# biotite-dev/springcraft

Hardware: AMD Instinct MI355X
Metric: ANM modes/sec (Hessian build + full eigensolve), N=2000 C-alpha (higher is better)
Workload: dtype f64; 1 GPU; C3: N=2000 C-alpha ANM, HinsenForceField (no cutoff), full 6000x6000 eigensolve, all modes + vectors; parallelism=independent structures sharded over GPUs, no data-path collective

## Files before the change

### springcraft_amd/csrc/host_logic.h

```cpp
#pragma once
#include <cmath>
#include <cstdarg>
#include <cstdint>
#include <cstdio>
#include <map>
#include <string>
#include <utility>
#include <vector>

#include "scratch_arena.h"
#include "springcraft_hip.h"

namespace sc_host {

static inline int fail(std::string& err, int code, const char* fmt, ...) {
  char buf[512];
  va_list ap;
  va_start(ap, fmt);
  vsnprintf(buf, sizeof(buf), fmt, ap);
  va_end(ap);
  err = buf;
  return code;
}

static inline int check_ff(const sc_ff_desc* ff, std::string& err) {
  if (!ff) return fail(err, SC_ERR_INVALID_ARG, "force-field descriptor is NULL");
  if (ff->kind < SC_FF_INVARIANT || ff->kind > SC_FF_TABULATED)
    return fail(err, SC_ERR_INVALID_ARG, "unknown force-field kind %d", ff->kind);
  if (ff->kind == SC_FF_TABULATED) {
    const sc_tab_desc* t = ff->tab;
    if (!t || t->n_bins < 1 || !t->bonded || !t->intra_chain || !t->inter_chain || !t->atom_type || !t->chain ||
        !t->bonded_next || (t->n_bins > 1 && !t->edges_sq))
      return fail(err, SC_ERR_INVALID_ARG, "incomplete tabulated force-field descriptor");
  }
  if (ff->kind == SC_FF_INVARIANT && !ff->has_cutoff)
    return fail(err, SC_ERR_INVALID_ARG, "Cutoff distance must be a float");
  return SC_OK;
}

struct HostPatch {
  bool any = false;
  std::vector<uint8_t> shut;
  std::vector<int32_t> row_ptr, col;
  std::vector<int8_t> flag;
  std::vector<double> gam;
  int mask_gamma = 0;
  struct Bufs { uint8_t* shut; int32_t* rp; int32_t* col; int8_t* flag; double* gam; };
  Bufs layout(Arena& a) const {
    return Bufs{a.take<uint8_t>(shut.size()), a.take<int32_t>(row_ptr.size()), a.take<int32_t>(col.size() + 1),
                a.take<int8_t>(flag.size() + 1), a.take<double>(gam.size() + 1)};
  }
  size_t device_bytes() const {
    Arena a;
    layout(a);
    return a.bytes();
  }
};

static inline int build_patch(const sc_patch_desc* pd, int64_t n, HostPatch& hp, std::string& err) {
  hp.any = false;
  if (!pd || (pd->n_shutdown == 0 && pd->n_pair_off == 0 && pd->n_pair_on == 0)) return SC_OK;
  if (pd->n_shutdown < 0 || pd->n_pair_off < 0 || pd->n_pair_on < 0 ||
      (pd->n_shutdown && !pd->shutdown) || (pd->n_pair_off && !pd->pair_off) ||
      (pd->n_pair_on && !pd->pair_on))
    return fail(err, SC_ERR_INVALID_ARG, "inconsistent patch descriptor");
  hp.any = true;
  hp.mask_gamma = pd->base_cutoff_masks_gamma;
  hp.shut.assign((size_t)n, 0);
  auto in_range = [&](int64_t v) { return v >= 0 && v < n; };
  for (int64_t s = 0; s < pd->n_shutdown; ++s) {
    if (!in_range(pd->shutdown[s]))
      return fail(err, SC_ERR_INDEX, "Index %lld is out of bounds for a structure of length %lld",
                          (long long)pd->shutdown[s], (long long)n);
    hp.shut[(size_t)pd->shutdown[s]] = 1;
  }
  struct Ov { int8_t flag; double gam; };
  std::map<std::pair<int32_t, int32_t>, Ov> ov;
  auto touch = [&](int64_t i, int64_t j) -> Ov& {
    auto key = std::make_pair((int32_t)i, (int32_t)j);
    auto it = ov.find(key);
    if (it == ov.end()) it = ov.emplace(key, Ov{0, -1.0}).first;
    return it->second;
  };
  for (int64_t p = 0; p < pd->n_pair_off; ++p) {
    const int64_t i = pd->pair_off[2 * p], j = pd->pair_off[2 * p + 1];
    if (!in_range(i) || !in_range(j))
      return fail(err, SC_ERR_INDEX, "Index %lld is out of bounds for a structure of length %lld",
                          (long long)(in_range(i) ? j : i), (long long)n);
    touch(i, j).flag = 0;
    touch(j, i).flag = 0;
  }
  for (int64_t p = 0; p < pd->n_pair_on; ++p) {
    const int64_t i = pd->pair_on[2 * p], j = pd->pair_on[2 * p + 1];
    if (!in_range(i) || !in_range(j))
      return fail(err, SC_ERR_INDEX, "Index %lld is out of bounds for a structure of length %lld",
                          (long long)(in_range(i) ? j : i), (long long)n);
    if (i == j)
      return fail(err, SC_ERR_SELF_PAIR, "Cannot turn on interaction of an atom with itself");
  }
  for (int pass = 0; pass < 2; ++pass)
    for (int64_t p = 0; p < pd->n_pair_on; ++p) {
      const int64_t i = pd->pair_on[2 * p + pass], j = pd->pair_on[2 * p + 1 - pass];
      Ov& o = touch(i, j);
      o.flag = 1;
      if (pd->on_force_constants) o.gam = pd->on_force_constants[p];
    }
  hp.row_ptr.assign((size_t)n + 1, 0);
  for (auto& kv : ov) hp.row_ptr[(size_t)kv.first.first + 1]++;
  for (int64_t i = 0; i < n; ++i) hp.row_ptr[i + 1] += hp.row_ptr[i];
  hp.col.reserve(ov.size());
  hp.flag.reserve(ov.size());
  hp.gam.reserve(ov.size());
  for (auto& kv : ov) {
    hp.col.push_back(kv.first.second);
    hp.flag.push_back(kv.second.flag);
    hp.gam.push_back(kv.second.gam == -1.0 ? std::nan("") : kv.second.gam);
  }
  return SC_OK;
}


constexpr int kResidentRowsLds = 8, kResidentRowsReg = 12;
constexpr int kResidentMaxLds = 2048, kResidentMaxReg = 3072;
constexpr int kResidentSmallDoubles = 160;
constexpr int kResidentMinOrder = 128;
struct ResidentShape {
  int off, m;
  int P, logP;
  int Q;
  bool reg;
  size_t lds_bytes;
};
static inline bool resident_shape(int n, int nb, int cus, int max_order, int want_wgs, ResidentShape* out) {
  if (n < kResidentMinOrder || nb <= 0) return false;
  int max_m = cus >= 256 ? kResidentMaxReg : kResidentMaxLds;
  if (max_order >= kResidentMinOrder && max_order < max_m) max_m = max_order;
  ResidentShape R{};
  R.off = n > max_m ? (n - max_m + nb - 1) / nb * nb : 0;
  R.m = n - R.off;
  if (R.m < kResidentMinOrder) return false;
  R.reg = R.m > kResidentMaxLds;
  const int rows = R.reg ? kResidentRowsReg : kResidentRowsLds;
  int P = 32, lp = 5;
  while ((R.m + P - 1) / P > rows) { P *= 2; ++lp; }
  while (P < want_wgs && 2 * P <= 256) { P *= 2; ++lp; }
  if (P > cus || P > 256) return false;
  R.P = P;
  R.logP = lp;
  const int qn = (R.m + 255) / 256;
  R.Q = R.reg ? (qn <= 10 ? 10 : 12) : (qn <= 2 ? qn : (qn <= 4 ? 4 : (qn <= 6 ? 6 : 8)));
  const size_t rmax = (size_t)(R.m - 1) / P + 1;
  R.lds_bytes = sizeof(double) * ((R.reg ? 0 : rmax * 256 * R.Q) + kResidentSmallDoubles);
  *out = R;
  return true;
}

}
```

### springcraft_amd/csrc/stedc.hip

```cpp
#include <algorithm>
#include <vector>

#include "eigh_internal.h"

namespace {

constexpr double kEps = 2.220446049250313e-16;

__device__ __forceinline__ int* iptr(double* ws, long long off) { return reinterpret_cast<int*>(ws + off); }
__device__ __forceinline__ const int* iptr(const double* ws, long long off) {
  return reinterpret_cast<const int*>(ws + off);
}

__device__ __forceinline__ double wave_sum_all(double v) {
#pragma unroll
  for (int off = 32; off > 0; off >>= 1) v += __shfl_xor(v, off);
  return v;
}
__device__ __forceinline__ double wave_prod_all(double v) {
#pragma unroll
  for (int off = 32; off > 0; off >>= 1) v *= __shfl_xor(v, off);
  return v;
}
__device__ __forceinline__ double wave_max_all(double v) {
#pragma unroll
  for (int off = 32; off > 0; off >>= 1) v = fmax(v, __shfl_xor(v, off));
  return v;
}

__global__ void k_dc_prepare(const double* __restrict__ tri_all, TriLayout TL, double* __restrict__ dc_all,
                             DcLayout DL, const DcNode* __restrict__ nodes, int n_nodes) {
  __shared__ double red[16];
  const double* tri = tri_all + (size_t)blockIdx.x * TL.slab;
  double* ws = dc_all + (size_t)blockIdx.x * DL.slab;
  const int n = DL.n, tid = threadIdx.x;
  double mx = 0.0;
  for (int i = tid; i < n; i += blockDim.x) {
    mx = fmax(mx, fabs(tri[TL.d + i]));
    if (i < n - 1) mx = fmax(mx, fabs(tri[TL.e + i]));
  }
  mx = wave_max_all(mx);
  if ((tid & 63) == 0) red[tid >> 6] = mx;
  __syncthreads();
  mx = 0.0;
  for (int w = 0; w < (int)(blockDim.x >> 6); ++w) mx = fmax(mx, red[w]);
  const double nrm = (mx > 0.0 && mx == mx) ? mx : 1.0;
  const double inv = 1.0 / nrm;
  for (int i = tid; i < n; i += blockDim.x) {
    const double dv = tri[TL.d + i] * inv;
    const double ev = (i < n - 1) ? tri[TL.e + i] * inv : 0.0;
    ws[DL.dd + i] = fabs(dv) < 1e-150 ? 0.0 : dv;
    ws[DL.ee + i] = fabs(ev) < 1e-150 ? 0.0 : ev;
  }
  if (tid == 0) ws[DL.scale] = nrm;
  __syncthreads();
  for (int g = tid; g < n_nodes; g += blockDim.x) {
    const int mid = nodes[g].mid;
    const double r = fabs(ws[DL.ee + mid - 1]);
    ws[DL.dd + mid - 1] -= r;
    ws[DL.dd + mid] -= r;
  }
}

template <int LEAF>
__global__ __launch_bounds__(64) void k_dc_leaves(double* __restrict__ dc_all, DcLayout DL,
                                                  const DcNode* __restrict__ leaves,
                                                  double* __restrict__ q_all, long long stride_q,
                                                  int* __restrict__ fail_flag) {
  __shared__ double Z[LEAF][LEAF + 1];
  __shared__ double d[LEAF], e[LEAF];
  double* ws = dc_all + (size_t)blockIdx.y * DL.slab;
  double* Q = q_all + (size_t)blockIdx.y * stride_q;
  const int lo = leaves[blockIdx.x].lo, hi = leaves[blockIdx.x].hi;
  const int s = hi - lo, n = DL.n;
  const int lane = threadIdx.x;
  if (lane < s) {
    for (int c = 0; c < s; ++c) Z[lane][c] = (c == lane) ? 1.0 : 0.0;
    d[lane] = ws[DL.dd + lo + lane];
    e[lane] = (lane < s - 1) ? ws[DL.ee + lo + lane] : 0.0;
  }
  __syncthreads();
  for (int l = 0; l < s; ++l) {
    int iter = 0;
    int m;
    do {
      for (m = l; m < s - 1; ++m) {
        const double dd = fabs(d[m]) + fabs(d[m + 1]);
        if (fabs(e[m]) <= kEps * dd) break;
      }
      if (m != l) {
        if (++iter > 80) {
          if (lane == 0) atomicExch(fail_flag, 1);
          break;
        }
        double g = (d[l + 1] - d[l]) / (2.0 * e[l]);
        double r = hypot(g, 1.0);
        g = d[m] - d[l] + e[l] / (g + copysign(r, g));
        double sn = 1.0, cs = 1.0, p = 0.0;
        int i;
        for (i = m - 1; i >= l; --i) {
          double f = sn * e[i];
          const double b = cs * e[i];
          r = hypot(f, g);
          __syncthreads();
          e[i + 1] = r;
          if (r == 0.0) {
            d[i + 1] -= p;
            e[m] = 0.0;
            __syncthreads();
            break;
          }
          sn = f / r;
          cs = g / r;
          g = d[i + 1] - p;
          r = (d[i] - g) * sn + 2.0 * cs * b;
          p = sn * r;
          d[i + 1] = g + p;
          g = cs * r - b;
          if (lane < s) {
            f = Z[lane][i + 1];
            Z[lane][i + 1] = sn * Z[lane][i] + cs * f;
            Z[lane][i] = cs * Z[lane][i] - sn * f;
          }
          __syncthreads();
        }
        if (r == 0.0 && i >= l) continue;
        __syncthreads();
        d[l] -= p;
        e[l] = g;
        e[m] = 0.0;
        __syncthreads();
      }
    } while (m != l);
  }
  __syncthreads();
  for (int a = 0; a < s - 1; ++a) {
    int k = a;
    double best = d[a];
    for (int b = a + 1; b < s; ++b)
      if (d[b] < best) { best = d[b]; k = b; }
    __syncthreads();
    if (k != a) {
      const double tmp = d[a];
      __syncthreads();
      d[k] = tmp;
      d[a] = best;
      if (lane < s) {
        const double t2 = Z[lane][a];
        Z[lane][a] = Z[lane][k];
        Z[lane][k] = t2;
      }
    }
    __syncthreads();
  }
  if (lane < s) {
    ws[DL.w0 + lo + lane] = d[lane];
    for (int c = 0; c < s; ++c) Q[(size_t)(lo + c) * n + lo + lane] = Z[lane][c];
  }
}

__global__ void k_dc_zero_offdiag(const DcNode* __restrict__ nodes, double* __restrict__ q_all,
                                  long long stride_q, int n) {
  const DcNode nd = nodes[blockIdx.y];
  double* Q = q_all + (size_t)blockIdx.z * stride_q;
  const int n1 = nd.mid - nd.lo, n2 = nd.hi - nd.mid;
  const long long total = 2LL * n1 * n2;
  for (long long idx = blockIdx.x * (long long)blockDim.x + threadIdx.x; idx < total;
       idx += (long long)gridDim.x * blockDim.x) {
    if (idx < (long long)n1 * n2) {
      const int r = nd.mid + (int)(idx % n2), c = nd.lo + (int)(idx / n2);
      Q[(size_t)c * n + r] = 0.0;
    } else {
      const long long k = idx - (long long)n1 * n2;
      const int r = nd.lo + (int)(k % n1), c = nd.mid + (int)(k / n1);
      Q[(size_t)c * n + r] = 0.0;
    }
  }
}

__global__ __launch_bounds__(1024) void k_dc_setup(double* __restrict__ dc_all, DcLayout DL,
                                                   const DcNode* __restrict__ nodes, int nodes_in_level,
                                                   const double* __restrict__ q_all, long long stride_q,
                                                   long long w_old_off, GemmDesc* __restrict__ descs,
                                                   int use_lds, double* __restrict__ gscratch,
                                                   long long gscratch_stride) {
  extern __shared__ __attribute__((aligned(16))) double lds[];
  __shared__ double red[16];
  __shared__ double s_tol;
  const int g = blockIdx.x, b = blockIdx.y;
  const DcNode nd = nodes[g];
  double* ws = dc_all + (size_t)b * DL.slab;
  const double* Q = q_all + (size_t)b * stride_q;
  const int n = DL.n, lo = nd.lo, mid = nd.mid, hi = nd.hi;
  const int N = hi - lo, n1 = mid - lo;
  const int tid = threadIdx.x, nthr = blockDim.x;
  const double* wold = ws + w_old_off;

  double* sd;
  double* sz;
  int* scol;
  unsigned char* smix;
  unsigned char* sflag;
  if (use_lds) {
    sd = lds;
    sz = lds + N;
    scol = reinterpret_cast<int*>(lds + 2 * N);
    smix = reinterpret_cast<unsigned char*>(scol + N);
  } else {
    double* base = gscratch + (size_t)b * gscratch_stride + 3LL * lo;
    sd = base;
    sz = base + N;
    scol = reinterpret_cast<int*>(base + 2 * N);
    smix = reinterpret_cast<unsigned char*>(scol + N);
  }
  sflag = smix + N;

  const double rho_raw = ws[DL.ee + mid - 1];
  const double sgn = rho_raw < 0.0 ? -1.0 : 1.0;
  const double rho = 2.0 * fabs(rho_raw);
  const double isq2 = 0.7071067811865475244;

  double zmax = 0.0, dmax = 0.0;
  for (int j = tid; j < N; j += nthr) {
    const int col = lo + j;
    const double zj = (j < n1 ? Q[(size_t)col * n + (mid - 1)] : sgn * Q[(size_t)col * n + mid]) * isq2;
    ws[DL.z + col] = zj;
    zmax = fmax(zmax, fabs(zj));
    dmax = fmax(dmax, fabs(wold[col]));
  }
  zmax = wave_max_all(zmax);
  dmax = wave_max_all(dmax);
  if ((tid & 63) == 0) red[tid >> 6] = fmax(zmax, dmax);
  __syncthreads();
  if (tid == 0) {
    double mx = 0.0;
    for (int w = 0; w < (nthr >> 6); ++w) mx = fmax(mx, red[w]);
    s_tol = 8.0 * kEps * mx;
  }
  __syncthreads();
  for (int j = tid; j < N; j += nthr) {
    const double v = wold[lo + j];
    int rank;
    if (j < n1) {
      int a = 0, c = N - n1;
      while (a < c) {
        const int h = (a + c) >> 1;
        if (wold[mid + h] < v) a = h + 1; else c = h;
      }
      rank = j + a;
    } else {
      int a = 0, c = n1;
      while (a < c) {
        const int h = (a + c) >> 1;
        if (wold[lo + h] <= v) a = h + 1; else c = h;
      }
      rank = (j - n1) + a;
    }
    sd[rank] = v;
    sz[rank] = ws[DL.z + lo + j];
    scol[rank] = lo + j;
    smix[rank] = 0;
  }
  __syncthreads();

  const double tol = s_tol;
  int* src = iptr(ws, DL.src);
  int* rot_a = iptr(ws, DL.rot_a);
  int* rot_b = iptr(ws, DL.rot_b);
  int* cnt = iptr(ws, DL.cnt);
  int* ktop_src = iptr(ws, DL.ktop_src);
  int* ktop_k = iptr(ws, DL.ktop_k);
  int* kbot_src = iptr(ws, DL.kbot_src);
  int* kbot_k = iptr(ws, DL.kbot_k);
  __shared__ int wsum[3][16];
  __shared__ int s_nrot;
  const int L = (N + nthr - 1) / nthr;
  const int j0 = min(tid * L, N), j1 = min(j0 + L, N);

  for (int j = tid; j < N; j += nthr) sflag[j] = !(rho * fabs(sz[j]) > tol) ? 1 : 0;
  if (tid == 0) s_nrot = 0;
  __syncthreads();
  int nseed = 0;
  for (int jj = j0; jj < j1; ++jj) {
    if (sflag[jj] & 1) continue;
    int pj = jj - 1;
    while (pj >= 0 && (sflag[pj] & 1)) --pj;
    if (pj < 0) continue;
    double s = sz[pj], c = sz[jj];
    const double tau = hypot(c, s);
    const double t = sd[jj] - sd[pj];
    c /= tau;
    s /= tau;
    if (fabs(t * c * s) <= tol) { sflag[jj] |= 2; ++nseed; }
  }
  const int any_rot = __syncthreads_or(nseed);
  if (any_rot) {
    int is = nseed;
    for (int off = 1; off < 64; off <<= 1) {
      const int us = __shfl_up(is, off);
      if ((tid & 63) >= off) is += us;
    }
    if ((tid & 63) == 63) wsum[0][tid >> 6] = is;
    __syncthreads();
    int bs = 0, total = 0;
    for (int w = 0; w < (nthr >> 6); ++w) {
      if (w < (tid >> 6)) bs += wsum[0][w];
      total += wsum[0][w];
    }
    int pos = bs + is - nseed;
    for (int jj = j0; jj < j1; ++jj)
      if (sflag[jj] & 2) kbot_k[lo + pos++] = jj;
    __syncthreads();
    if (tid == 0) {
      int nrot = 0, done_upto = -1;
      for (int si = 0; si < total; ++si) {
        int jj = kbot_k[lo + si];
        if (jj <= done_upto) continue;
        int pj = jj - 1;
        while (pj >= 0 && (sflag[pj] & 5)) --pj;
        while (true) {
          double s = sz[pj], c = sz[jj];
          const double tau = hypot(c, s);
          const double t = sd[jj] - sd[pj];
          c /= tau;
          s /= tau;
          done_upto = jj;
          if (!(fabs(t * c * s) <= tol)) break;
          sz[jj] = tau;
          sz[pj] = 0.0;
          rot_a[lo + nrot] = scol[pj];
          rot_b[lo + nrot] = scol[jj];
          ws[DL.rot_c + lo + nrot] = c;
// ... 122 lines not shown
  }
  const int lane = threadIdx.x & 63;
  const int j = blockIdx.x * waves + (threadIdx.x >> 6);
  if (j >= K) return;
  const double rho = 2.0 * fabs(ws[DL.ee + nd.mid - 1]);
  const double rinv = 1.0 / rho;

  auto fsum2 = [&](double dorg, double tau, double& fp) -> double {
    double s = 0.0, sp = 0.0;
    if (z2) {
      for (int i = lane; i < K; i += 64) {
        const double r = 1.0 / ((dl[i] - dorg) - tau);
        const double zr = z2[i] * r;
        s += zr;
        sp += zr * r;
      }
    } else {
      for (int i = lane; i < K; i += 64) {
        const double z = zzg[i];
        const double r = 1.0 / ((dl[i] - dorg) - tau);
        const double zr = z * z * r;
        s += zr;
        sp += zr * r;
      }
    }
    fp = wave_sum_all(sp);
    return rinv + wave_sum_all(s);
  };
  auto fsum = [&](double dorg, double tau) -> double {
    double fp;
    return fsum2(dorg, tau, fp);
  };

  int org;
  bool positive;
  double t_hi;
  double t_start = 0.0;
  double zj2 = 0.0, zk2 = 0.0;
  if (j == K - 1) {
    org = K - 1;
    positive = true;
    double s2 = 0.0;
    if (z2) { for (int i = lane; i < K; i += 64) s2 += z2[i]; }
    else { for (int i = lane; i < K; i += 64) s2 += zzg[i] * zzg[i]; }
    s2 = wave_sum_all(s2);
    t_hi = rho * s2 * (1.0 + 8.0 * kEps) + 1e-300;
  } else {
    const double gap = dl[j + 1] - dl[j];
    const double half = 0.5 * gap;
    const double fm = fsum(dl[j], half);
    if (fm > 0.0) { org = j; positive = true; } else { org = j + 1; positive = false; }
    t_hi = half;
    {
      zj2 = z2 ? z2[j] : zzg[j] * zzg[j];
      zk2 = z2 ? z2[j + 1] : zzg[j + 1] * zzg[j + 1];
      const double c = fm + (zj2 - zk2) / half;
      double t0;
      if (positive) {
        const double a = c * gap + zj2 + zk2, b = zj2 * gap;
        const double disc = sqrt(fabs(a * a - 4.0 * b * c));
        t0 = a > 0.0 ? 2.0 * b / (a + disc) : (a - disc) / (2.0 * c);
      } else {
        const double a = c * gap - zj2 - zk2, b = zk2 * gap;
        const double disc = sqrt(fabs(a * a + 4.0 * b * c));
        t0 = -(a < 0.0 ? 2.0 * b / (a - disc) : -(a + disc) / (2.0 * c));
      }
      if (t0 == t0 && t0 > 0.0 && t0 < t_hi) t_start = t0;
    }
  }
  const double dorg = dl[org];
  unsigned long long lo_b = 0ull, hi_b = (unsigned long long)__double_as_longlong(t_hi);
  unsigned long long t_b = hi_b - ((hi_b - lo_b) >> 1);
  if (t_start > 0.0) t_b = (unsigned long long)__double_as_longlong(t_start);
  unsigned long long probe_dist = 4ull;
  double t_accept = 0.0;
  for (int it = 0; it < 90 && hi_b - lo_b > 1ull; ++it) {
    const double t = __longlong_as_double((long long)t_b);
    double fp;
    const double f = fsum2(dorg, positive ? t : -t, fp);
    const bool go_up = positive ? (f < 0.0) : (f > 0.0);
    if (go_up) lo_b = t_b; else hi_b = t_b;
    if (hi_b - lo_b <= 1ull) break;
    const unsigned long long mid_b = lo_b + ((hi_b - lo_b) >> 1);
    double tn;
    bool model_step = false;
    if (j < K - 1 && fabs(f) * t < 0.25 * (positive ? zj2 : zk2)) {
      model_step = true;
      const double tau = positive ? t : -t;
      const double dj = (dl[j] - dorg) - tau, dk = (dl[j + 1] - dorg) - tau;
      const double dw = fp;
      double c;
      if (positive) {
        const double q = zj2 / (dj * dj);
        c = f - dk * dw - (dl[j] - dl[j + 1]) * q;
      } else {
        const double q = zk2 / (dk * dk);
        c = f - dj * dw - (dl[j + 1] - dl[j]) * q;
      }
      const double a = (dj + dk) * f - dj * dk * dw;
      const double b = dj * dk * f;
      double eta;
      if (c == 0.0) {
        eta = a != 0.0 ? b / a : -f / dw;
      } else {
        const double disc = sqrt(fabs(a * a - 4.0 * b * c));
        eta = a <= 0.0 ? (a - disc) / (2.0 * c) : 2.0 * b / (a + disc);
      }
      if (f * eta >= 0.0) eta = -f / dw;
      const double tau_n = tau + eta;
      tn = positive ? tau_n : -tau_n;
    } else {
      const double fpt = positive ? fp : -fp;
      const double den = fpt * t + f;
      tn = fpt * t * t / den;
    }
    unsigned long long n_b = mid_b;
    if (tn == tn && tn > 0.0 && tn < 1.7e308) {
      const unsigned long long c_b = (unsigned long long)__double_as_longlong(tn);
      if (c_b > lo_b && c_b < hi_b) {
        n_b = c_b;
        const unsigned long long step = c_b > t_b ? c_b - t_b : t_b - c_b;
#ifndef DC_STRICT_BRACKET
        if (step <= 2ull || (model_step && fabs(tn - t) <= 1e-12 * t)) {
          t_accept = tn;
          break;
        }
#endif
        if (step <= 4ull) {
          const unsigned long long far = go_up ? c_b + probe_dist : (c_b > probe_dist ? c_b - probe_dist : 0ull);
          n_b = (far > lo_b && far < hi_b) ? far : mid_b;
          probe_dist *= 8ull;
        }
      }
    }
    t_b = n_b;
  }
  double t_best = __longlong_as_double((long long)hi_b);
  if (t_accept > 0.0) {
    t_best = t_accept;
  } else if (lo_b > 0ull) {
    const double t_lo = __longlong_as_double((long long)lo_b);
    const double f_lo = fabs(fsum(dorg, positive ? t_lo : -t_lo));
    const double f_hi = fabs(fsum(dorg, positive ? t_best : -t_best));
    if (f_lo < f_hi) t_best = t_lo;
  }
  if (lane == 0) {
    const double tau = positive ? t_best : -t_best;
    iptr(ws, DL.org)[lo + j] = org;
    ws[DL.tauv + lo + j] = tau;
    ws[DL.lam + lo + j] = dorg + tau;
  }
}

__global__ __launch_bounds__(256) void k_dc_zhat(double* __restrict__ dc_all, DcLayout DL,
                                                 const DcNode* __restrict__ nodes) {
  const int g = blockIdx.y, b = blockIdx.z;
  const DcNode nd = nodes[g];
  double* ws = dc_all + (size_t)b * DL.slab;
  const int K = iptr(ws, DL.cnt)[2 * g];
  const int i = blockIdx.x * (blockDim.x >> 6) + (threadIdx.x >> 6);
  if (i >= K) return;
  const int lane = threadIdx.x & 63, lo = nd.lo;
  const double* dl = ws + DL.dl + lo;
  const int* org = iptr(ws, DL.org) + lo;
  const double* tauv = ws + DL.tauv + lo;
  const double di = dl[i];
  double prod = 1.0;
  for (int j = lane; j < K; j += 64) {
    const double num = (di - dl[org[j]]) - tauv[j];
    prod *= (j == i) ? num : num / (di - dl[j]);
  }
  prod = wave_prod_all(prod);
  if (lane == 0) ws[DL.zhat + lo + i] = copysign(sqrt(fabs(prod)), ws[DL.zz + lo + i]);
}

__global__ __launch_bounds__(256) void k_dc_vectors(double* __restrict__ dc_all, DcLayout DL,
                                                    const DcNode* __restrict__ nodes,
                                                    double* __restrict__ u_all, long long stride_u) {
  __shared__ double red[4];
  const int g = blockIdx.y, b = blockIdx.z;
  const DcNode nd = nodes[g];
  double* ws = dc_all + (size_t)b * DL.slab;
  const int K = iptr(ws, DL.cnt)[2 * g];
  const int j = blockIdx.x;
  if (j >= K) return;
  const int lo = nd.lo, n = DL.n;
  const double* dl = ws + DL.dl + lo;
  const double* zh = ws + DL.zhat + lo;
  const double dorg = dl[iptr(ws, DL.org)[lo + j]];
  const double tau = ws[DL.tauv + lo + j];
  double* U = u_all + (size_t)b * stride_u + (size_t)(lo + j) * n + lo;
  double ss = 0.0;
  for (int i = threadIdx.x; i < K; i += blockDim.x) {
    const double u = zh[i] / ((dl[i] - dorg) - tau);
    U[i] = u;
    ss += u * u;
  }
  ss = wave_sum_all(ss);
  if ((threadIdx.x & 63) == 0) red[threadIdx.x >> 6] = ss;
  __syncthreads();
  const double inv = 1.0 / sqrt((red[0] + red[1]) + (red[2] + red[3]));
  for (int i = threadIdx.x; i < K; i += blockDim.x) U[i] *= inv;
}

__global__ __launch_bounds__(256) void k_dc_finalize(double* __restrict__ dc_all, DcLayout DL,
                                                     const DcNode* __restrict__ nodes, long long w_new_off) {
  const int g = blockIdx.y, b = blockIdx.z;
  const DcNode nd = nodes[g];
  double* ws = dc_all + (size_t)b * DL.slab;
  const int K = iptr(ws, DL.cnt)[2 * g];
  const int lo = nd.lo, hi = nd.hi, N = hi - lo, ndef = N - K;
  const int idx = blockIdx.x * blockDim.x + threadIdx.x;
  if (idx >= N) return;
  const double* lam = ws + DL.lam + lo;
  int* dest = iptr(ws, DL.dest);
  double* wnew = ws + w_new_off;
  auto defval = [&](int e) { return ws[DL.ddef + hi - 1 - e]; };
  if (idx < K) {
    const double v = lam[idx];
    int c = 0;
    for (int e = 0; e < ndef; ++e) c += defval(e) < v;
    dest[lo + idx] = lo + idx + c;
    wnew[lo + idx + c] = v;
  } else {
    const int e = idx - K;
    const double v = defval(e);
    int a = 0, c = K;
    while (a < c) {
      const int h = (a + c) >> 1;
      if (lam[h] <= v) a = h + 1; else c = h;
    }
    int r = a;
    for (int f = 0; f < ndef; ++f) {
      const double u = defval(f);
      r += (u < v) || (u == v && f < e);
    }
    dest[lo + idx] = lo + r;
    wnew[lo + r] = v;
  }
}

__global__ __launch_bounds__(256) void k_dc_copy_deflated(double* __restrict__ dc_all, DcLayout DL,
                                                          const DcNode* __restrict__ nodes,
                                                          const double* __restrict__ q_old_all,
                                                          double* __restrict__ q_new_all,
                                                          long long stride_q) {
  const int g = blockIdx.y, b = blockIdx.z;
  const DcNode nd = nodes[g];
  double* ws = dc_all + (size_t)b * DL.slab;
  const int K = iptr(ws, DL.cnt)[2 * g];
  const int lo = nd.lo, hi = nd.hi, N = hi - lo;
  const int e = blockIdx.x;
  if (e >= N - K) return;
  const int n = DL.n;
  const int scol = iptr(ws, DL.src)[hi - 1 - e];
  const int dcol = iptr(ws, DL.dest)[lo + K + e];
  const double* qs = q_old_all + (size_t)b * stride_q + (size_t)scol * n + lo;
  double* qd = q_new_all + (size_t)b * stride_q + (size_t)dcol * n + lo;
  for (int r = threadIdx.x; r < N; r += blockDim.x) qd[r] = qs[r];
}

__global__ void k_dc_unscale(const double* __restrict__ dc_all, DcLayout DL, long long w_off,
                             double* __restrict__ w_out, long long stride_w) {
  const double* ws = dc_all + (size_t)blockIdx.y * DL.slab;
  const int i = blockIdx.x * blockDim.x + threadIdx.x;
  if (i < DL.n) w_out[(size_t)blockIdx.y * stride_w + i] = ws[w_off + i] * ws[DL.scale];
}

struct Tree {
  std::vector<DcNode> leaves;
  std::vector<std::vector<DcNode>> levels;
};

Tree build_tree(int n, int leaf_max) {
  int depth = 0;
  while (((n + (1 << depth) - 1) >> depth) > leaf_max) ++depth;
  std::vector<std::vector<DcNode>> by_depth(depth + 1);
  by_depth[0].push_back(DcNode{0, n / 2, n});
  for (int dlev = 0; dlev < depth; ++dlev) {
    for (const DcNode& nd : by_depth[dlev]) {
      by_depth[dlev + 1].push_back(DcNode{nd.lo, nd.lo + (nd.mid - nd.lo) / 2, nd.mid});
      by_depth[dlev + 1].push_back(DcNode{nd.mid, nd.mid + (nd.hi - nd.mid) / 2, nd.hi});
    }
  }
  Tree t;
  t.leaves = by_depth[depth];
  for (int dlev = depth - 1; dlev >= 0; --dlev) t.levels.push_back(by_depth[dlev]);
  return t;
}

constexpr int kLeafMax = 32;
constexpr int kLdsCapSetup = 7000;
constexpr int kLdsCapSecular = 9800;

}

int dc_max_nodes(int n, int leaf_max) {
  Tree t = build_tree(n, leaf_max);
  size_t total = t.leaves.size();
  for (auto& l : t.levels) total += l.size();
  return (int)total;
}

size_t dc_slab_doubles(int n, DcLayout* out) {
  DcLayout L{};
  L.n = n;
  L.leaf_max = kLeafMax;
  long long off = 0;
  const long long nn = ((long long)n + 7) / 8 * 8;
  auto take = [&](long long cnt) { long long o = off; off += (cnt + 7) / 8 * 8; return o; };
  L.dd = take(nn); L.ee = take(nn); L.w0 = take(nn); L.w1 = take(nn); L.z = take(nn);
  L.dl = take(nn); L.zz = take(nn); L.ddef = take(nn); L.lam = take(nn); L.tauv = take(nn);
  L.zhat = take(nn); L.rot_c = take(nn); L.rot_s = take(nn); L.scale = take(8);
  L.src = take(nn); L.org = take(nn); L.dest = take(nn); L.rot_a = take(nn); L.rot_b = take(nn);
  L.ktop_src = take(nn); L.ktop_k = take(nn); L.kbot_src = take(nn); L.kbot_k = take(nn);
  L.cnt = take(2LL * dc_max_nodes(n, kLeafMax) + 8);
  L.slab = off;
  if (out) *out = L;
  return (size_t)off;
}

__global__ __launch_bounds__(1024) void k_dc_desc_flops(const GemmDesc* __restrict__ d, int count, double* __restrict__ out) {
  __shared__ double part[16];
  double a = 0.0;
  for (int r = threadIdx.x; r < count; r += 1024) a += 2.0 * (double)d[r].m * (double)d[r].n * (double)d[r].k;
#pragma unroll
  for (int off = 32; off > 0; off >>= 1) a += __shfl_xor(a, off);
  if ((threadIdx.x & 63) == 0) part[threadIdx.x >> 6] = a;
  __syncthreads();
  if (threadIdx.x == 0) {
    double t = 0.0;
    for (int w = 0; w < 16; ++w) t += part[w];
    *out = t;
  }
}

int stedc_batched(sc_ctx* ctx, int n, int batch, const double* d_tri_ws, const TriLayout& TL,
                  double* d_dc_ws, const DcLayout& DL, double* d_w, long long stride_w, double* d_q_out,
                  double* d_q_tmp, double* d_u, long long stride_q, GemmDesc* d_merge_descs) {
  hipStream_t st = ctx->stream;
  Tree tree = build_tree(n, kLeafMax);
  const int nlev = (int)tree.levels.size();

  std::vector<DcNode> flat(tree.leaves);
  std::vector<size_t> lev_off(nlev);
  for (int l = 0; l < nlev; ++l) {
    lev_off[l] = flat.size();
    flat.insert(flat.end(), tree.levels[l].begin(), tree.levels[l].end());
  }
  const size_t n_internal = flat.size() - tree.leaves.size();
  const size_t node_bytes = align_up(flat.size() * sizeof(DcNode), 256);
  const size_t big_bytes = n > kLdsCapSetup ? (size_t)batch * 3 * n * sizeof(double) : 0;
  SC_TRY(sc_reserve_dc_aux(ctx, node_bytes + 256 + big_bytes));
  DcNode* d_nodes = reinterpret_cast<DcNode*>(ctx->dc_aux);
  int* d_fail = reinterpret_cast<int*>(ctx->d_status + 1);
  double* d_big = big_bytes ? reinterpret_cast<double*>(reinterpret_cast<char*>(d_nodes) + node_bytes + 256) : nullptr;
  SC_TRY(sc_stage_upload(ctx, d_nodes, flat.data(), flat.size() * sizeof(DcNode)));

  auto qbuf = [&](int stage) { return ((nlev - stage) % 2 == 0) ? d_q_out : d_q_tmp; };

  std::vector<GemmDesc> h_descs;
  std::vector<size_t> desc_off(nlev);
  for (int l = 0; l < nlev; ++l) {
    desc_off[l] = h_descs.size();
    const auto& nodes = tree.levels[l];
    const double* q_old = qbuf(l);
    double* q_new = qbuf(l + 1);
    for (int b = 0; b < batch; ++b)
      for (size_t g = 0; g < nodes.size(); ++g) {
        const DcNode& nd = nodes[g];
        auto ip = [&](long long off) { return reinterpret_cast<const int*>(d_dc_ws + (size_t)b * DL.slab + off) + nd.lo; };
        for (int half = 0; half < 2; ++half) {
          const int r0 = half == 0 ? nd.lo : nd.mid;
          GemmDesc D{};
          D.a = q_old + (size_t)b * stride_q + r0;
          D.sa_i = 1; D.sa_k = n;
          D.a_kidx = ip(half == 0 ? DL.ktop_src : DL.kbot_src);
          D.b = d_u + (size_t)b * stride_q + (size_t)nd.lo * n + nd.lo;
          D.sb_k = 1; D.sb_j = n;
          D.b_kidx = ip(half == 0 ? DL.ktop_k : DL.kbot_k);
          D.c = q_new + (size_t)b * stride_q + r0;
          D.ldc = n;
          D.c_jidx = ip(DL.dest);
          D.m = half == 0 ? nd.mid - nd.lo : nd.hi - nd.mid; D.n = 0; D.k = 0;
          D.alpha = 1.0; D.beta = 0.0;
          h_descs.push_back(D);
        }
      }
  }
  if (!h_descs.empty()) SC_TRY(sc_stage_upload(ctx, d_merge_descs, h_descs.data(), h_descs.size() * sizeof(GemmDesc)));

  hipLaunchKernelGGL(k_dc_prepare, dim3((unsigned)batch), dim3(1024), 0, st, d_tri_ws, TL, d_dc_ws, DL,
                     d_nodes + tree.leaves.size(), (int)n_internal);
  hipLaunchKernelGGL((k_dc_leaves<kLeafMax>), dim3((unsigned)tree.leaves.size(), (unsigned)batch), dim3(64),
                     0, st, d_dc_ws, DL, d_nodes, qbuf(0), stride_q, d_fail);

  PhaseTimer t_gemm(ctx, "dc_gemm", st);
  for (int l = 0; l < nlev; ++l) {
    const auto& nodes = tree.levels[l];
    const int G = (int)nodes.size();
    const DcNode* dn = d_nodes + lev_off[l];
    int maxN = 0;
    for (auto& nd : nodes) maxN = std::max(maxN, nd.hi - nd.lo);
    double* q_old = qbuf(l);
    double* q_new = qbuf(l + 1);
    const long long w_old = (l % 2 == 0) ? DL.w0 : DL.w1;
    const long long w_new = (l % 2 == 0) ? DL.w1 : DL.w0;
    GemmDesc* descs = d_merge_descs + desc_off[l];

    hipLaunchKernelGGL(k_dc_zero_offdiag,
                       dim3((unsigned)std::min(1024, (maxN * maxN / 2 + 255) / 256 + 1), (unsigned)G,
                            (unsigned)batch),
                       dim3(256), 0, st, dn, q_old, stride_q, n);
    {
      const int use_lds = maxN <= kLdsCapSetup ? 1 : 0;
      const size_t lds = use_lds ? (size_t)maxN * 22 + 32 : 0;
      const int threads = maxN >= 1024 ? 1024 : (maxN >= 256 ? 256 : 64);
      hipLaunchKernelGGL(k_dc_setup, dim3((unsigned)G, (unsigned)batch), dim3(threads), lds, st, d_dc_ws, DL,
                         dn, G, q_old, stride_q, w_old, descs, use_lds, d_big, (long long)3 * n);
    }
    hipLaunchKernelGGL(k_dc_rotate, dim3((unsigned)((maxN + 255) / 256), (unsigned)G, (unsigned)batch),
                       dim3(256), 0, st, d_dc_ws, DL, dn, q_old, stride_q);
    {
      const int use_lds = maxN <= kLdsCapSecular ? 1 : 0;
      const int threads = maxN >= 2048 ? 1024 : 256;
      const int waves = threads / 64;
      const size_t lds = use_lds ? (size_t)maxN * 16 + 16 : 0;
      hipLaunchKernelGGL(k_dc_secular, dim3((unsigned)((maxN + waves - 1) / waves), (unsigned)G, (unsigned)batch),
                         dim3(threads), lds, st, d_dc_ws, DL, dn, use_lds);
    }
    hipLaunchKernelGGL(k_dc_zhat, dim3((unsigned)((maxN + 3) / 4), (unsigned)G, (unsigned)batch), dim3(256), 0,
                       st, d_dc_ws, DL, dn);
    hipLaunchKernelGGL(k_dc_vectors, dim3((unsigned)maxN, (unsigned)G, (unsigned)batch), dim3(256), 0, st,
                       d_dc_ws, DL, dn, d_u, stride_q);
    hipLaunchKernelGGL(k_dc_finalize, dim3((unsigned)((maxN + 255) / 256), (unsigned)G, (unsigned)batch),
                       dim3(256), 0, st, d_dc_ws, DL, dn, w_new);
    hipLaunchKernelGGL(k_dc_copy_deflated, dim3((unsigned)maxN, (unsigned)G, (unsigned)batch), dim3(256), 0, st,
                       d_dc_ws, DL, dn, q_old, q_new, stride_q);
    t_gemm.start();
    SC_TRY(launch_gemm_f64(ctx, descs, {.count = 2 * G * batch, .max_m = (maxN + 1) / 2, .max_n = maxN, .layout = kGemmAmBk, .gather = true}));
    t_gemm.stop();
  }
  const long long w_final = (nlev % 2 == 0) ? DL.w0 : DL.w1;
  hipLaunchKernelGGL(k_dc_unscale, dim3((unsigned)((n + 255) / 256), (unsigned)batch), dim3(256), 0, st,
                     d_dc_ws, DL, w_final, d_w, stride_w);
  SC_HIP(ctx, hipGetLastError());

  t_gemm.finish();
  if (ctx->profiling && !h_descs.empty()) {
    double* d_flops = reinterpret_cast<double*>(reinterpret_cast<char*>(d_nodes) + node_bytes);
    hipLaunchKernelGGL(k_dc_desc_flops, dim3(1), dim3(1024), 0, st, d_merge_descs, (int)h_descs.size(), d_flops);
    double h_flops = 0.0;
    SC_HIP(ctx, hipMemcpyAsync(&h_flops, d_flops, sizeof(double), hipMemcpyDeviceToHost, st));
    SC_HIP(ctx, hipStreamSynchronize(st));
    bool found = false;
    for (auto& ph : ctx->phases)
      if (ph.first == "dc_gemm_gflop") { ph.second = h_flops * 1e-9; found = true; }
    if (!found) ctx->phases.emplace_back("dc_gemm_gflop", h_flops * 1e-9);
  }
  return SC_OK;
}
```

Baseline: 178,900 modes/s.

## Streamline divide-and-conquer merge chain: targeted column zeroing, register vectors, batched zhat

Behind a default-on environment switch, the full off-diagonal block zeroing of Q is replaced by a kernel that zeros only the deflated and rotated columns after setup. The zhat product kernel now handles four roots per wave, and eigenvector formation keeps entries in registers instead of re-reading them. A multi-root secular solver is also added, but the default root count is 1, so the original secular kernel still runs. The goal is to cut memory traffic and launch work in each merge level, at the cost of more template variants and correctness depending on which columns are skipped.

Result: no change. 179,700 modes/s, median of 6 (+0.5%).

```diff
diff --git a/springcraft_amd/csrc/host_logic.h b/springcraft_amd/csrc/host_logic.h
--- a/springcraft_amd/csrc/host_logic.h
+++ b/springcraft_amd/csrc/host_logic.h
@@ -155,4 +155,42 @@
   return true;
 }
 
+#ifndef SC_DC_VEC_REG_MAX
+#define SC_DC_VEC_REG_MAX 24
+#endif
+constexpr int kDcVecThreads = 256;
+constexpr int kDcVecRegMax = SC_DC_VEC_REG_MAX;
+constexpr int kDcLdsCapSecular = 9800;
+constexpr int kDcSecularRoots = 1, kDcZhatPerWave = 4;
+struct DcChainShape {
+  int vec_regs;
+  int sec_threads, sec_roots, sec_use_lds;
+  unsigned sec_grid_x;
+  size_t sec_lds_bytes;
+  int zhat_per_wave;
+  unsigned zhat_grid_x;
+};
+static inline DcChainShape dc_chain_shape(int maxN, bool chain, int roots_override = 0) {
+  DcChainShape S{};
+  const int per_thread = (maxN + kDcVecThreads - 1) / kDcVecThreads;
+  S.vec_regs = 0;
+  if (chain)
+    for (int r : {4, 8, 16, 24})
+      if (per_thread <= r && r <= kDcVecRegMax) { S.vec_regs = r; break; }
+  S.sec_use_lds = maxN <= kDcLdsCapSecular ? 1 : 0;
+  S.sec_threads = maxN >= 2048 ? 1024 : 256;
+  S.sec_roots = 1;
+  if (chain && S.sec_use_lds) {
+    S.sec_roots = kDcSecularRoots;
+    if (roots_override == 1 || roots_override == 2 || roots_override == 4) S.sec_roots = roots_override;
+    if (S.sec_roots == 4 && S.sec_threads == 1024) S.sec_roots = 2;
+  }
+  const int per_wg = S.sec_threads / 64 * S.sec_roots;
+  S.sec_grid_x = (unsigned)((maxN + per_wg - 1) / per_wg);
+  S.sec_lds_bytes = S.sec_use_lds ? (size_t)maxN * 16 + 16 : 0;
+  S.zhat_per_wave = chain ? kDcZhatPerWave : 1;
+  S.zhat_grid_x = (unsigned)((maxN + 4 * S.zhat_per_wave - 1) / (4 * S.zhat_per_wave));
+  return S;
 }
+
+}
diff --git a/springcraft_amd/csrc/stedc.hip b/springcraft_amd/csrc/stedc.hip
--- a/springcraft_amd/csrc/stedc.hip
+++ b/springcraft_amd/csrc/stedc.hip
@@ -1,7 +1,9 @@
 #include <algorithm>
+#include <cstdlib>
 #include <vector>
 
 #include "eigh_internal.h"
+#include "host_logic.h"
 
 namespace {
 
@@ -178,6 +180,29 @@
   }
 }
 
+__global__ __launch_bounds__(256) void k_dc_zero_cols(const double* __restrict__ dc_all, DcLayout DL,
+                                                      const DcNode* __restrict__ nodes, double* __restrict__ q_all,
+                                                      long long stride_q) {
+  const int g = blockIdx.y, b = blockIdx.z;
+  const DcNode nd = nodes[g];
+  const double* ws = dc_all + (size_t)b * DL.slab;
+  const int K = iptr(ws, DL.cnt)[2 * g], nrot = iptr(ws, DL.cnt)[2 * g + 1];
+  const int lo = nd.lo, mid = nd.mid, hi = nd.hi;
+  const int e = blockIdx.x;
+  if (e >= (hi - lo) - K) return;
+  double* Q = q_all + (size_t)b * stride_q;
+  const int n = DL.n;
+  const int cols[2] = {iptr(ws, DL.src)[hi - 1 - e], e < nrot ? iptr(ws, DL.rot_b)[lo + e] : -1};
+#pragma unroll
+  for (int s = 0; s < 2; ++s) {
+    const int c = cols[s];
+    if (c < 0) continue;
+    const int r0 = c < mid ? mid : lo, r1 = c < mid ? hi : mid;
+    double* q = Q + (size_t)c * n;
+    for (int r = r0 + (int)threadIdx.x; r < r1; r += blockDim.x) q[r] = 0.0;
+  }
+}
+
 __global__ __launch_bounds__(1024) void k_dc_setup(double* __restrict__ dc_all, DcLayout DL,
                                                    const DcNode* __restrict__ nodes, int nodes_in_level,
                                                    const double* __restrict__ q_all, long long stride_q,
@@ -606,6 +631,240 @@
   }
 }
 
+template <int R, int THREADS>
+__global__ __launch_bounds__(THREADS) void k_dc_secular_multi(double* __restrict__ dc_all, DcLayout DL,
+                                                              const DcNode* __restrict__ nodes) {
+  extern __shared__ __attribute__((aligned(16))) double lds[];
+  const int g = blockIdx.y, b = blockIdx.z;
+  const DcNode nd = nodes[g];
+  double* ws = dc_all + (size_t)b * DL.slab;
+  const int K = iptr(ws, DL.cnt)[2 * g];
+  constexpr int waves = THREADS >> 6;
+  if ((int)blockIdx.x * waves * R >= K) return;
+  const int lo = nd.lo;
+  {
+    const double* dlg = ws + DL.dl + lo;
+    const double* zzg = ws + DL.zz + lo;
+    for (int i = threadIdx.x; i < K; i += THREADS) {
+      lds[i] = dlg[i];
+      const double z = zzg[i];
+      lds[K + i] = z * z;
+    }
+  }
+  __syncthreads();
+  const double* dl = lds;
+  const double* z2 = lds + K;
+  const int lane = threadIdx.x & 63;
+  const int j0 = (blockIdx.x * waves + (threadIdx.x >> 6)) * R;
+  if (j0 >= K) return;
+  const double rho = 2.0 * fabs(ws[DL.ee + nd.mid - 1]);
+  const double rinv = 1.0 / rho;
+
+  auto fsum2 = [&](const double (&dorg)[R], const double (&tau)[R], double (&f)[R], double (&fp)[R]) __attribute__((always_inline)) {
+    double s[R], sp[R];
+#pragma unroll
+    for (int r = 0; r < R; ++r) { s[r] = 0.0; sp[r] = 0.0; }
+    for (int i = lane; i < K; i += 64) {
+      const double di = dl[i], zi = z2[i];
+#pragma unroll
+      for (int r = 0; r < R; ++r) {
+        const double q = 1.0 / ((di - dorg[r]) - tau[r]);
+        const double zr = zi * q;
+        s[r] += zr;
+        sp[r] += zr * q;
+      }
+    }
+#pragma unroll
+    for (int r = 0; r < R; ++r) {
+      fp[r] = wave_sum_all(sp[r]);
+      f[r] = rinv + wave_sum_all(s[r]);
+    }
+  };
+  auto fsum = [&](const double (&dorg)[R], const double (&tau)[R], double (&f)[R]) __attribute__((always_inline)) {
+    double fp[R];
+    fsum2(dorg, tau, f, fp);
+  };
+
+  int jr[R], org[R];
+  bool valid[R], edge[R], positive[R];
+  double t_hi[R], t_start[R], zj2[R], zk2[R], dorg[R], targ[R], fv[R], fpv[R];
+#pragma unroll
+  for (int r = 0; r < R; ++r) {
+    jr[r] = j0 + r;
+    valid[r] = jr[r] < K;
+    edge[r] = jr[r] == K - 1;
+    org[r] = K - 1;
+    positive[r] = true;
+    t_hi[r] = 1.0;
+    t_start[r] = 0.0;
+    zj2[r] = 0.0;
+    zk2[r] = 0.0;
+    const bool interior = valid[r] && !edge[r];
+    dorg[r] = dl[interior ? jr[r] : K - 1];
+    targ[r] = interior ? 0.5 * (dl[jr[r] + 1] - dl[jr[r]]) : 1.0;
+  }
+  bool any_edge = false;
+#pragma unroll
+  for (int r = 0; r < R; ++r) any_edge = any_edge || edge[r];
+  if (any_edge) {
+    double s2 = 0.0;
+    for (int i = lane; i < K; i += 64) s2 += z2[i];
+    s2 = wave_sum_all(s2);
+#pragma unroll
+    for (int r = 0; r < R; ++r)
+      if (edge[r]) t_hi[r] = rho * s2 * (1.0 + 8.0 * kEps) + 1e-300;
+  }
+  bool any_interior = false;
+#pragma unroll
+  for (int r = 0; r < R; ++r) any_interior = any_interior || (valid[r] && !edge[r]);
+  if (any_interior) fsum(dorg, targ, fv);
+#pragma unroll
+  for (int r = 0; r < R; ++r) {
+    if (!(valid[r] && !edge[r])) continue;
+    const int j = jr[r];
+    const double gap = dl[j + 1] - dl[j];
+    const double half = 0.5 * gap;
+    const double fm = fv[r];
+    if (fm > 0.0) { org[r] = j; positive[r] = true; } else { org[r] = j + 1; positive[r] = false; }
+    t_hi[r] = half;
+    {
+      zj2[r] = z2[j];
+      zk2[r] = z2[j + 1];
+      const double c = fm + (zj2[r] - zk2[r]) / half;
+      double t0;
+      if (positive[r]) {
+        const double a = c * gap + zj2[r] + zk2[r], b = zj2[r] * gap;
+        const double disc = sqrt(fabs(a * a - 4.0 * b * c));
+        t0 = a > 0.0 ? 2.0 * b / (a + disc) : (a - disc) / (2.0 * c);
+      } else {
+        const double a = c * gap - zj2[r] - zk2[r], b = zk2[r] * gap;
+        const double disc = sqrt(fabs(a * a + 4.0 * b * c));
+        t0 = -(a < 0.0 ? 2.0 * b / (a - disc) : -(a + disc) / (2.0 * c));
+      }
+      if (t0 == t0 && t0 > 0.0 && t0 < t_hi[r]) t_start[r] = t0;
+    }
+  }
+  unsigned long long lo_b[R], hi_b[R], t_b[R], probe_dist[R];
+  double t_accept[R];
+  bool alive[R];
+#pragma unroll
+  for (int r = 0; r < R; ++r) {
+    dorg[r] = dl[org[r]];
+    lo_b[r] = 0ull;
+    hi_b[r] = (unsigned long long)__double_as_longlong(t_hi[r]);
+    t_b[r] = hi_b[r] - ((hi_b[r] - lo_b[r]) >> 1);
+    if (t_start[r] > 0.0) t_b[r] = (unsigned long long)__double_as_longlong(t_start[r]);
+    probe_dist[r] = 4ull;
+    t_accept[r] = 0.0;
+    alive[r] = valid[r];
+  }
+  auto step = [&](int r, double f, double fp) __attribute__((always_inline)) {
+    const int j = jr[r];
+    const double t = __longlong_as_double((long long)t_b[r]);
+    const bool go_up = positive[r] ? (f < 0.0) : (f > 0.0);
+    if (go_up) lo_b[r] = t_b[r]; else hi_b[r] = t_b[r];
+    if (hi_b[r] - lo_b[r] <= 1ull) { alive[r] = false; return; }
+    const unsigned long long mid_b = lo_b[r] + ((hi_b[r] - lo_b[r]) >> 1);
+    double tn;
+    bool model_step = false;
+    if (j < K - 1 && fabs(f) * t < 0.25 * (positive[r] ? zj2[r] : zk2[r])) {
+      model_step = true;
+      const double tau = positive[r] ? t : -t;
+      const double dj = (dl[j] - dorg[r]) - tau, dk = (dl[j + 1] - dorg[r]) - tau;
+      const double dw = fp;
+      double c;
+      if (positive[r]) {
+        const double q = zj2[r] / (dj * dj);
+        c = f - dk * dw - (dl[j] - dl[j + 1]) * q;
+      } else {
+        const double q = zk2[r] / (dk * dk);
+        c = f - dj * dw - (dl[j + 1] - dl[j]) * q;
+      }
+      const double a = (dj + dk) * f - dj * dk * dw;
+      const double b = dj * dk * f;
+      double eta;
+      if (c == 0.0) {
+        eta = a != 0.0 ? b / a : -f / dw;
+      } else {
+        const double disc = sqrt(fabs(a * a - 4.0 * b * c));
+        eta = a <= 0.0 ? (a - disc) / (2.0 * c) : 2.0 * b / (a + disc);
+      }
+      if (f * eta >= 0.0) eta = -f / dw;
+      const double tau_n = tau + eta;
+      tn = positive[r] ? tau_n : -tau_n;
+    } else {
+      const double fpt = positive[r] ? fp : -fp;
+      const double den = fpt * t + f;
+      tn = fpt * t * t / den;
+    }
+    unsigned long long n_b = mid_b;
+    if (tn == tn && tn > 0.0 && tn < 1.7e308) {
+      const unsigned long long c_b = (unsigned long long)__double_as_longlong(tn);
+      if (c_b > lo_b[r] && c_b < hi_b[r]) {
+        n_b = c_b;
+        const unsigned long long stp = c_b > t_b[r] ? c_b - t_b[r] : t_b[r] - c_b;
+#ifndef DC_STRICT_BRACKET
+        if (stp <= 2ull || (model_step && fabs(tn - t) <= 1e-12 * t)) {
+          t_accept[r] = tn;
+          alive[r] = false;
+          return;
+        }
+#endif
+        if (stp <= 4ull) {
+          const unsigned long long far = go_up ? c_b + probe_dist[r] : (c_b > probe_dist[r] ? c_b - probe_dist[r] : 0ull);
+          n_b = (far > lo_b[r] && far < hi_b[r]) ? far : mid_b;
+          probe_dist[r] *= 8ull;
+        }
+      }
+    }
+    t_b[r] = n_b;
+  };
+  for (int it = 0; it < 90; ++it) {
+    bool any = false;
+#pragma unroll
+    for (int r = 0; r < R; ++r) {
+      alive[r] = alive[r] && (hi_b[r] - lo_b[r] > 1ull);
+      any = any || alive[r];
+      const double t = __longlong_as_double((long long)t_b[r]);
+      targ[r] = positive[r] ? t : -t;
+    }
+    if (!any) break;
+    fsum2(dorg, targ, fv, fpv);
+#pragma unroll
+    for (int r = 0; r < R; ++r)
+      if (alive[r]) step(r, fv[r], fpv[r]);
+  }
+  double t_best[R], t_lo[R];
+  bool need[R], any_need = false;
+#pragma unroll
+  for (int r = 0; r < R; ++r) {
+    t_best[r] = __longlong_as_double((long long)hi_b[r]);
+    need[r] = valid[r] && !(t_accept[r] > 0.0) && lo_b[r] > 0ull;
+    any_need = any_need || need[r];
+    t_lo[r] = __longlong_as_double((long long)(need[r] ? lo_b[r] : hi_b[r]));
+  }
+  if (any_need) {
+    double f_lo[R], f_hi[R], a_lo[R], a_hi[R];
+#pragma unroll
+    for (int r = 0; r < R; ++r) { a_lo[r] = positive[r] ? t_lo[r] : -t_lo[r]; a_hi[r] = positive[r] ? t_best[r] : -t_best[r]; }
+    fsum(dorg, a_lo, f_lo);
+    fsum(dorg, a_hi, f_hi);
+#pragma unroll
+    for (int r = 0; r < R; ++r)
+      if (need[r] && fabs(f_lo[r]) < fabs(f_hi[r])) t_best[r] = t_lo[r];
+  }
+#pragma unroll
+  for (int r = 0; r < R; ++r) {
+    if (t_accept[r] > 0.0) t_best[r] = t_accept[r];
+    if (lane == 0 && valid[r]) {
+      const double tau = positive[r] ? t_best[r] : -t_best[r];
+      iptr(ws, DL.org)[lo + jr[r]] = org[r];
+      ws[DL.tauv + lo + jr[r]] = tau;
+      ws[DL.lam + lo + jr[r]] = dorg[r] + tau;
+    }
+  }
+}
+
 __global__ __launch_bounds__(256) void k_dc_zhat(double* __restrict__ dc_all, DcLayout DL,
                                                  const DcNode* __restrict__ nodes) {
   const int g = blockIdx.y, b = blockIdx.z;
@@ -626,6 +885,42 @@
   }
   prod = wave_prod_all(prod);
   if (lane == 0) ws[DL.zhat + lo + i] = copysign(sqrt(fabs(prod)), ws[DL.zz + lo + i]);
+}
+
+template <int R>
+__global__ __launch_bounds__(256) void k_dc_zhat_multi(double* __restrict__ dc_all, DcLayout DL,
+                                                       const DcNode* __restrict__ nodes) {
+  const int g = blockIdx.y, b = blockIdx.z;
+  const DcNode nd = nodes[g];
+  double* ws = dc_all + (size_t)b * DL.slab;
+  const int K = iptr(ws, DL.cnt)[2 * g];
+  const int i0 = (blockIdx.x * (blockDim.x >> 6) + (threadIdx.x >> 6)) * R;
+  if (i0 >= K) return;
+  const int lane = threadIdx.x & 63, lo = nd.lo;
+  const double* dl = ws + DL.dl + lo;
+  const int* org = iptr(ws, DL.org) + lo;
+  const double* tauv = ws + DL.tauv + lo;
+  int ii[R];
+  double di[R], prod[R];
+#pragma unroll
+  for (int r = 0; r < R; ++r) {
+    ii[r] = min(i0 + r, K - 1);
+    di[r] = dl[ii[r]];
+    prod[r] = 1.0;
+  }
+  for (int j = lane; j < K; j += 64) {
+    const double dorg = dl[org[j]], tj = tauv[j], dj = dl[j];
+#pragma unroll
+    for (int r = 0; r < R; ++r) {
+      const double num = (di[r] - dorg) - tj;
+      prod[r] *= (j == ii[r]) ? num : num / (di[r] - dj);
+    }
+  }
+#pragma unroll
+  for (int r = 0; r < R; ++r) {
+    const double p = wave_prod_all(prod[r]);
+    if (lane == 0 && i0 + r < K) ws[DL.zhat + lo + i0 + r] = copysign(sqrt(fabs(p)), ws[DL.zz + lo + i0 + r]);
+  }
 }
 
 __global__ __launch_bounds__(256) void k_dc_vectors(double* __restrict__ dc_all, DcLayout DL,
@@ -655,6 +950,52 @@
   __syncthreads();
   const double inv = 1.0 / sqrt((red[0] + red[1]) + (red[2] + red[3]));
   for (int i = threadIdx.x; i < K; i += blockDim.x) U[i] *= inv;
+}
+
+template <int NT>
+__global__ __launch_bounds__(256) void k_dc_vectors_reg(double* __restrict__ dc_all, DcLayout DL,
+                                                        const DcNode* __restrict__ nodes,
+                                                        double* __restrict__ u_all, long long stride_u) {
+  __shared__ double red[4];
+  const int g = blockIdx.y, b = blockIdx.z;
+  const DcNode nd = nodes[g];
+  double* ws = dc_all + (size_t)b * DL.slab;
+  const int K = iptr(ws, DL.cnt)[2 * g];
+  const int j = blockIdx.x;
+  if (j >= K) return;
+  const int lo = nd.lo, n = DL.n;
+  const double* dl = ws + DL.dl + lo;
+  const double* zh = ws + DL.zhat + lo;
+  const double dorg = dl[iptr(ws, DL.org)[lo + j]];
+  const double tau = ws[DL.tauv + lo + j];
+  double* U = u_all + (size_t)b * stride_u + (size_t)(lo + j) * n + lo;
+  double a[NT], z[NT], u[NT];
+#pragma unroll
+  for (int t = 0; t < NT; ++t) {
+    const int i = min(t * 256 + (int)threadIdx.x, K - 1);
+    a[t] = dl[i];
+    z[t] = zh[i];
+  }
+  double ss = 0.0;
+#pragma unroll
+  for (int t = 0; t < NT; ++t) {
+    u[t] = 0.0;
+    if (t * 256 < K) {
+      if (t * 256 + (int)threadIdx.x < K) {
+        u[t] = z[t] / ((a[t] - dorg) - tau);
+        ss += u[t] * u[t];
+      }
+    }
+  }
+  ss = wave_sum_all(ss);
+  if ((threadIdx.x & 63) == 0) red[threadIdx.x >> 6] = ss;
+  __syncthreads();
+  const double inv = 1.0 / sqrt((red[0] + red[1]) + (red[2] + red[3]));
+#pragma unroll
+  for (int t = 0; t < NT; ++t) {
+    const int i = t * 256 + (int)threadIdx.x;
+    if (i < K) U[i] = u[t] * inv;
+  }
 }
 
 __global__ __launch_bounds__(256) void k_dc_finalize(double* __restrict__ dc_all, DcLayout DL,
@@ -745,7 +1086,6 @@
 
 constexpr int kLeafMax = 32;
 constexpr int kLdsCapSetup = 7000;
-constexpr int kLdsCapSecular = 9800;
 
 }
 
@@ -849,6 +1189,8 @@
   hipLaunchKernelGGL((k_dc_leaves<kLeafMax>), dim3((unsigned)tree.leaves.size(), (unsigned)batch), dim3(64),
                      0, st, d_dc_ws, DL, d_nodes, qbuf(0), stride_q, d_fail);
 
+  const bool chain = [] { const char* e = getenv("SPRINGCRAFT_DC_CHAIN"); return !(e && atoi(e) == 0); }();
+  const int env_roots = [] { const char* e = getenv("SPRINGCRAFT_DC_ROOTS"); return e ? atoi(e) : 0; }();
   PhaseTimer t_gemm(ctx, "dc_gemm", st);
   for (int l = 0; l < nlev; ++l) {
     const auto& nodes = tree.levels[l];
@@ -862,10 +1204,12 @@
     const long long w_new = (l % 2 == 0) ? DL.w1 : DL.w0;
     GemmDesc* descs = d_merge_descs + desc_off[l];
 
-    hipLaunchKernelGGL(k_dc_zero_offdiag,
-                       dim3((unsigned)std::min(1024, (maxN * maxN / 2 + 255) / 256 + 1), (unsigned)G,
-                            (unsigned)batch),
-                       dim3(256), 0, st, dn, q_old, stride_q, n);
+    const sc_host::DcChainShape S = sc_host::dc_chain_shape(maxN, chain, env_roots);
+    if (!chain)
+      hipLaunchKernelGGL(k_dc_zero_offdiag,
+                         dim3((unsigned)std::min(1024, (maxN * maxN / 2 + 255) / 256 + 1), (unsigned)G,
+                              (unsigned)batch),
+                         dim3(256), 0, st, dn, q_old, stride_q, n);
     {
       const int use_lds = maxN <= kLdsCapSetup ? 1 : 0;
       const size_t lds = use_lds ? (size_t)maxN * 22 + 32 : 0;
@@ -873,20 +1217,39 @@
       hipLaunchKernelGGL(k_dc_setup, dim3((unsigned)G, (unsigned)batch), dim3(threads), lds, st, d_dc_ws, DL,
                          dn, G, q_old, stride_q, w_old, descs, use_lds, d_big, (long long)3 * n);
     }
+    if (chain)
+      hipLaunchKernelGGL(k_dc_zero_cols, dim3((unsigned)maxN, (unsigned)G, (unsigned)batch), dim3(256), 0, st, d_dc_ws,
+                         DL, dn, q_old, stride_q);
     hipLaunchKernelGGL(k_dc_rotate, dim3((unsigned)((maxN + 255) / 256), (unsigned)G, (unsigned)batch),
                        dim3(256), 0, st, d_dc_ws, DL, dn, q_old, stride_q);
     {
-      const int use_lds = maxN <= kLdsCapSecular ? 1 : 0;
-      const int threads = maxN >= 2048 ? 1024 : 256;
-      const int waves = threads / 64;
-      const size_t lds = use_lds ? (size_t)maxN * 16 + 16 : 0;
-      hipLaunchKernelGGL(k_dc_secular, dim3((unsigned)((maxN + waves - 1) / waves), (unsigned)G, (unsigned)batch),
-                         dim3(threads), lds, st, d_dc_ws, DL, dn, use_lds);
-    }
-    hipLaunchKernelGGL(k_dc_zhat, dim3((unsigned)((maxN + 3) / 4), (unsigned)G, (unsigned)batch), dim3(256), 0,
-                       st, d_dc_ws, DL, dn);
-    hipLaunchKernelGGL(k_dc_vectors, dim3((unsigned)maxN, (unsigned)G, (unsigned)batch), dim3(256), 0, st,
-                       d_dc_ws, DL, dn, d_u, stride_q);
+      const dim3 grid(S.sec_grid_x, (unsigned)G, (unsigned)batch);
+      auto multi = [&](void (*kern)(double*, DcLayout, const DcNode*), int threads) {
+        if (S.sec_lds_bytes > 64 * 1024)
+          sc_raise_dyn_lds(reinterpret_cast<const void*>(kern), 16 * sc_host::kDcLdsCapSecular + 16);
+        hipLaunchKernelGGL(kern, grid, dim3(threads), S.sec_lds_bytes, st, d_dc_ws, DL, dn);
+      };
+      if (S.sec_roots == 1)
+        hipLaunchKernelGGL(k_dc_secular, grid, dim3(S.sec_threads), S.sec_lds_bytes, st, d_dc_ws, DL, dn, S.sec_use_lds);
+      else if (S.sec_roots == 2 && S.sec_threads == 1024) multi(k_dc_secular_multi<2, 1024>, 1024);
+      else if (S.sec_roots == 2) multi(k_dc_secular_multi<2, 256>, 256);
+      else multi(k_dc_secular_multi<4, 256>, 256);
+    }
+    {
+      const dim3 grid(S.zhat_grid_x, (unsigned)G, (unsigned)batch);
+      if (S.zhat_per_wave == 1) hipLaunchKernelGGL(k_dc_zhat, grid, dim3(256), 0, st, d_dc_ws, DL, dn);
+      else hipLaunchKernelGGL((k_dc_zhat_multi<sc_host::kDcZhatPerWave>), grid, dim3(256), 0, st, d_dc_ws, DL, dn);
+    }
+    {
+      const dim3 grid((unsigned)maxN, (unsigned)G, (unsigned)batch);
+      switch (S.vec_regs) {
+        case 4: hipLaunchKernelGGL((k_dc_vectors_reg<4>), grid, dim3(256), 0, st, d_dc_ws, DL, dn, d_u, stride_q); break;
+        case 8: hipLaunchKernelGGL((k_dc_vectors_reg<8>), grid, dim3(256), 0, st, d_dc_ws, DL, dn, d_u, stride_q); break;
+        case 16: hipLaunchKernelGGL((k_dc_vectors_reg<16>), grid, dim3(256), 0, st, d_dc_ws, DL, dn, d_u, stride_q); break;
+        case 24: hipLaunchKernelGGL((k_dc_vectors_reg<24>), grid, dim3(256), 0, st, d_dc_ws, DL, dn, d_u, stride_q); break;
+        default: hipLaunchKernelGGL(k_dc_vectors, grid, dim3(256), 0, st, d_dc_ws, DL, dn, d_u, stride_q);
+      }
+    }
     hipLaunchKernelGGL(k_dc_finalize, dim3((unsigned)((maxN + 255) / 256), (unsigned)G, (unsigned)batch),
                        dim3(256), 0, st, d_dc_ws, DL, dn, w_new);
     hipLaunchKernelGGL(k_dc_copy_deflated, dim3((unsigned)maxN, (unsigned)G, (unsigned)batch), dim3(256), 0, st,
```
